# jpe17/TwoTowerMLRetrieval

Hardware: AMD Instinct MI355X
Metric: queries/sec top-k over 10M x 256-d docs (higher is better)
Workload: dtype f32 results (bit-identical to the fp32 FMA chain); f16-MFMA screen + fp32 rescoring; 1 GPU; exact cosine top-10 of B=1024 queries over 10000000 x 256 fp32 unit-norm passages resident in HBM (BASELINE configs[3]; configs[1] batch), row-sharded over 1 GPU(s), screened path (f16-MFMA filter + exact fp32 rescoring, bit-identical to the fp32 kernel); n_docs=10000000, dim=256, batch=1024, k=10, parallelism=rowshard1

## Files before the change

### twotowermlretrieval_amd/csrc/score_topk.hip

```cpp
#include "tt_common.h"

#include <limits.h>
#include <math.h>

namespace {

constexpr int TILE_DOCS = 32;
constexpr int SLAB_BYTES = 32 * 128;
constexpr int NSTAGE = 4;
#ifndef TT_K4_NT_NSTAGE
#define TT_K4_NT_NSTAGE 4
#endif
constexpr int NSTAGE_NT = TT_K4_NT_NSTAGE;
constexpr int WPB = 4;
constexpr int DMA_PER_SLAB = 4;
constexpr int PACE_R = 16;
constexpr int PACE_POLLS = 400;
constexpr int DRAW_POLLS = 1 << 16;
constexpr int DRAW_GAVE_UP = 0x7fffffff;

typedef __attribute__((address_space(3))) void lds_void;
typedef const __attribute__((address_space(1))) void gbl_void;

struct Cand;
// ... 692 lines not shown
            float bv;
            int64_t bi;
            pool_next_best(pool_v, pool_i, n, pv, pi, red_v, red_i, bv, bi);
            if (bi == INT64_MAX)
                break;
            if (tid == 0) {
                top_v[r] = bv;
                top_i[r] = bi;
            }
            pv = bv;
            pi = bi;
            kept = r + 1;
        }
        __syncthreads();
        if (tid < kept) {
            pool_v[tid] = top_v[tid];
            pool_i[tid] = top_i[tid];
        }
        if (tid == 0)
            pool_n = kept;
        __syncthreads();
        return kept;
    };

    for (int base = 0; base < M; base += MERGE_SEG) {
        if (pool_n + MERGE_SEG > MERGE_POOL)
            reduce_pool();
        const int end = min(base + MERGE_SEG, M);
        int64_t ci[MERGE_SEG / MERGE_THREADS];
#pragma unroll
        for (int u = 0; u < MERGE_SEG / MERGE_THREADS; ++u) {
            const int m = base + tid + u * MERGE_THREADS;
            ci[u] = m < end ? ix_at(m) : -1;
        }
#pragma unroll
        for (int u = 0; u < MERGE_SEG / MERGE_THREADS; ++u) {
            if (ci[u] >= 0) {
                const int slot = atomicAdd(&pool_n, 1);
                pool_v[slot] = v_at(base + tid + u * MERGE_THREADS);
                pool_i[slot] = ci[u];
            }
        }
        __syncthreads();
    }
    const int kept = reduce_pool();
    if (tid < k) {
        out_val[(size_t)b * k + tid] = tid < kept ? pool_v[tid] : -INFINITY;
        out_idx[(size_t)b * k + tid] = tid < kept ? pool_i[tid] : -1;
    }
}

__device__ __forceinline__ unsigned order_key(float f)
{
    const unsigned b = __float_as_uint(f);
    return (b & 0x80000000u) ? ~b : (b | 0x80000000u);
}

__device__ __forceinline__ float order_key_to_float(unsigned key)
{
    return __uint_as_float((key & 0x80000000u) ? (key & 0x7fffffffu) : ~key);
}

__global__ __launch_bounds__(256) void kth_largest_kernel(const float *__restrict__ vals, int M, int k,
                                                          float *__restrict__ out, const int *run_if,
                                                          float *__restrict__ top_out)
{
    if (run_if && run_if[blockIdx.x >> 5] == 0)
        return;
    __shared__ int hist[256];
    __shared__ int sel[2];
    __shared__ int wpos;
    const int row = blockIdx.x, tid = threadIdx.x, lane = tid & 63;
    const float *v = vals + (size_t)row * M;
    if (M < k) {
        if (tid == 0 && out)
            out[row] = -INFINITY;
        if (top_out)
            for (int i = tid; i < k; i += 256)
                top_out[(size_t)row * k + i] = i < M ? v[i] : -INFINITY;
        return;
    }
    unsigned prefix = 0u, mask = 0u;
    int k_rem = k;
    constexpr int KTH_REG = 16;
    const bool in_regs = M <= 256 * KTH_REG;
    unsigned keys[KTH_REG];
    if (in_regs) {
#pragma unroll
        for (int i = 0; i < KTH_REG; ++i) {
            const int m = tid + 256 * i;
            keys[i] = m < M ? order_key(v[m]) : 0u;
        }
    }
#pragma unroll 1
    for (int pass = 0; pass < 4; ++pass) {
        const int shift = 24 - 8 * pass;
        hist[tid] = 0;
        __syncthreads();
        if (in_regs) {
#pragma unroll
            for (int i = 0; i < KTH_REG; ++i)
                if (tid + 256 * i < M && (keys[i] & mask) == prefix)
                    atomicAdd(&hist[(keys[i] >> shift) & 255u], 1);
        } else {
            for (int m = tid; m < M; m += 256) {
                const unsigned key = order_key(v[m]);
                if ((key & mask) == prefix)
                    atomicAdd(&hist[(key >> shift) & 255u], 1);
            }
        }
        __syncthreads();
        if (tid < 64) {
            int c[4], s = 0;
#pragma unroll
            for (int i = 0; i < 4; ++i) {
                c[i] = hist[255 - (lane * 4 + i)];
                s += c[i];
            }
            int incl = s;
#pragma unroll
            for (int off = 1; off < 64; off <<= 1) {
                const int y = __shfl_up(incl, off);
                if (lane >= off)
                    incl += y;
            }
            int above = incl - s;
#pragma unroll
            for (int i = 0; i < 4; ++i) {
                if (above < k_rem && above + c[i] >= k_rem) {
                    sel[0] = 255 - (lane * 4 + i);
                    sel[1] = above;
                }
                above += c[i];
            }
        }
        __syncthreads();
        prefix |= (unsigned)sel[0] << shift;
        mask |= 0xffu << shift;
        k_rem -= sel[1];
        __syncthreads();
    }
    const float kth = order_key_to_float(prefix);
    if (tid == 0 && out)
        out[row] = kth;
    if (top_out) {
        if (tid == 0)
            wpos = 0;
        __syncthreads();
        float *dst = top_out + (size_t)row * k;
        if (in_regs) {
#pragma unroll
            for (int i = 0; i < KTH_REG; ++i)
                if (tid + 256 * i < M && keys[i] > prefix)
                    dst[atomicAdd(&wpos, 1)] = order_key_to_float(keys[i]);
        } else {
            for (int m = tid; m < M; m += 256)
                if (order_key(v[m]) > prefix)
                    dst[atomicAdd(&wpos, 1)] = v[m];
        }
        for (int i = k - k_rem + tid; i < k; i += 256)
            dst[i] = kth;
    }
}

__global__ __launch_bounds__(256) void score_rank_kernel(const float *__restrict__ Q,
                                                         const float *__restrict__ D, int N, int d,
                                                         const int64_t *__restrict__ target,
// ... 389 lines not shown
TT_EXPORT size_t tt_score_topk_redo_flags_offset(int B, int64_t N, int d, int k)
{
    if (B <= 0 || N <= 0 || k <= 0)
        return (size_t)-1;
    const Plan pl = make_plan(B, N, k, d);
    return (pl.paced && pl.main.tail_blocks > 0) ? pl.redo_off : (size_t)-1;
}

TT_EXPORT size_t tt_score_topk_workspace_bytes(int B, int64_t N, int d, int k)
{
    if (B <= 0 || N < 0 || k <= 0)
        return 0;
    return make_plan(B, N, k, d).ws_bytes;
}

TT_EXPORT size_t tt_score_topk_bf16_workspace_bytes(int B, int64_t N, int d, int k)
{
    if (B <= 0 || N < 0 || k <= 0)
        return 0;
    return make_plan(B, N, k, d, true).ws_bytes;
}

TT_EXPORT int tt_score_topk_partials_f32(const float *Q, int B, int d, const float *D, int64_t N, int k,
                                         int64_t idx_offset, void *workspace, size_t workspace_bytes,
                                         const float **part_val, const int64_t **part_idx, int *part_m,
                                         void *const *prof_events, tt_stream_t stream)
{
    Plan pl;
    int rc = score_partials(Q, B, d, D, false, N, k, idx_offset, workspace, workspace_bytes, (hipStream_t)stream, &pl,
                            "tt_score_topk_partials_f32", nullptr, prof_events);
    if (rc != TT_OK)
        return rc;
    if (part_val)
        *part_val = (const float *)((const char *)workspace + pl.pval_off);
    if (part_idx)
        *part_idx = (const int64_t *)((const char *)workspace + pl.pidx_off);
    if (part_m)
        *part_m = pl.main.n_chunks * k;
    return TT_OK;
}

namespace {
__global__ __launch_bounds__(64) void redo_flag_kernel(const int64_t *__restrict__ out_idx, int B, int k, int *__restrict__ flags)
{
    const int q = blockIdx.x * 32 + threadIdx.x;
    const bool bad = threadIdx.x < 32 && q < B && out_idx[(size_t)q * k] >= (int64_t)TT_TOPK_INVALID_INDEX;
    const unsigned long long any = __ballot(bad);
    if (threadIdx.x == 0)
        flags[blockIdx.x] = any != 0ull;
}
}

namespace {
int score_topk_pred(const float *Q, int B, int d, const void *D, bool bf16, int64_t N, int k, int64_t idx_offset,
                    float *out_val, int64_t *out_idx, void *workspace, size_t workspace_bytes, const int *run_if,
                    hipStream_t st, const char *who)
{
    if (B < 0 || N < 0 || k <= 0)
        return tt_fail(TT_ERR_BAD_SHAPE, "%s: B=%d N=%lld k=%d", who, B, (long long)N, k);
    if (B == 0)
        return TT_OK;
    if (!score_dim_ok(d, bf16))
        return tt_fail(TT_ERR_UNSUPPORTED, "%s: d=%d (supported: %s)", who, d, score_dims(bf16));
    if (k > 64)
        return tt_fail(TT_ERR_UNSUPPORTED, "%s: k=%d > 64", who, k);
    if (!out_val || !out_idx)
        return tt_fail(TT_ERR_BAD_SHAPE, "%s: null output pointer", who);
    if (N == 0) {
        hipLaunchKernelGGL(topk_merge_kernel, dim3(B), dim3(MERGE_THREADS), 0, st, (const float *)nullptr,
                           (const int64_t *)nullptr, 0, k, out_val, out_idx, (const int *)nullptr, 1, (size_t)0);
        TT_LAUNCH_CHECK();
        return TT_OK;
    }
    Plan pl;
    int rc = score_partials(Q, B, d, D, bf16, N, k, idx_offset, workspace, workspace_bytes, st, &pl, who, run_if);
    if (rc != TT_OK)
        return rc;
    const char *ws = (const char *)workspace;
    hipLaunchKernelGGL(topk_merge_kernel, dim3(B), dim3(MERGE_THREADS), 0, st, (const float *)(ws + pl.pval_off),
                       (const int64_t *)(ws + pl.pidx_off), pl.main.n_chunks * k, k, out_val, out_idx, run_if,
                       pl.main.n_chunks * k, (size_t)0);
    TT_LAUNCH_CHECK();
    if (!run_if && pl.paced && pl.main.tail_blocks > 0 && tt_score_pacing()) {
        int *redo = (int *)((char *)workspace + pl.redo_off);
        hipLaunchKernelGGL(redo_flag_kernel, dim3(pl.main.n_qtiles), dim3(64), 0, st, (const int64_t *)out_idx, B, k, redo);
        TT_LAUNCH_CHECK();
        return score_topk_pred(Q, B, d, D, bf16, N, k, idx_offset, out_val, out_idx, workspace, workspace_bytes, redo, st,
                               who);
    }
    return TT_OK;
}
}

int tt_score_topk_f32_pred(const float *Q, int B, int d, const float *D, int64_t N, int k, int64_t idx_offset,
                           float *out_val, int64_t *out_idx, void *workspace, size_t workspace_bytes,
                           const int *run_if, hipStream_t st)
{
    return score_topk_pred(Q, B, d, D, false, N, k, idx_offset, out_val, out_idx, workspace, workspace_bytes, run_if, st,
                           "tt_score_topk_f32");
}

int tt_score_topk_bf16_pred(const float *Q, int B, int d, const void *D, int64_t N, int k, int64_t idx_offset,
                            float *out_val, int64_t *out_idx, void *workspace, size_t workspace_bytes,
                            const int *run_if, hipStream_t st)
{
    return score_topk_pred(Q, B, d, D, true, N, k, idx_offset, out_val, out_idx, workspace, workspace_bytes, run_if, st,
                           "tt_score_topk_bf16");
}

TT_EXPORT int tt_score_topk_f32(const float *Q, int B, int d, const float *D, int64_t N, int k,
                                int64_t idx_offset, float *out_val, int64_t *out_idx, void *workspace,
                                size_t workspace_bytes, tt_stream_t stream)
{
    return tt_score_topk_f32_pred(Q, B, d, D, N, k, idx_offset, out_val, out_idx, workspace, workspace_bytes, nullptr,
                                  (hipStream_t)stream);
}

TT_EXPORT int tt_score_topk_bf16(const float *Q, int B, int d, const void *D_bf16, int64_t N, int k,
                                 int64_t idx_offset, float *out_val, int64_t *out_idx, void *workspace,
                                 size_t workspace_bytes, tt_stream_t stream)
{
    return tt_score_topk_bf16_pred(Q, B, d, D_bf16, N, k, idx_offset, out_val, out_idx, workspace, workspace_bytes,
                                   nullptr, (hipStream_t)stream);
}

int tt_kth_largest(const float *vals, int B, int M, int k, float *out, hipStream_t st)
{
    hipLaunchKernelGGL(kth_largest_kernel, dim3(B), dim3(256), 0, st, vals, M, k, out, (const int *)nullptr, (float *)nullptr);
    TT_LAUNCH_CHECK();
    return TT_OK;
}

int tt_k_largest_list(const float *vals, int B, int M, int k, float *list, hipStream_t st)
{
    hipLaunchKernelGGL(kth_largest_kernel, dim3(B), dim3(256), 0, st, vals, M, k, (float *)nullptr, (const int *)nullptr, list);
    TT_LAUNCH_CHECK();
    return TT_OK;
}

namespace {
__global__ __launch_bounds__(64) void seed_union_kernel(const float *__restrict__ lists, int world, int B, int ks, int kth,
                                                        float *__restrict__ seed)
{
    const int q = blockIdx.x, lane = threadIdx.x;
    const int M = world * ks;
    __shared__ float v[512];
    for (int i = lane; i < M; i += 64)
        v[i] = lists[((size_t)(i / ks) * B + q) * ks + (i % ks)];
    __syncthreads();
    for (int i = lane; i < M; i += 64) {
        const float x = v[i];
        int before = 0;
        for (int j = 0; j < M; ++j)
            before += (v[j] > x) || (v[j] == x && j < i);
        if (before == kth - 1)
            seed[q] = x;
    }
}
}

TT_EXPORT int tt_seed_union_f32(const float *lists, int world, int B, int list_len, int kth, float *seed, tt_stream_t stream)
{
    if (!lists || !seed || world < 1 || B <= 0 || list_len < 1 || (int64_t)world * list_len > 512 || kth < 1 ||
        kth > world * list_len)
        return tt_fail(TT_ERR_BAD_SHAPE, "tt_seed_union_f32: world=%d B=%d list_len=%d kth=%d (kth <= world * list_len <= 512)",
                       world, B, list_len, kth);
    hipLaunchKernelGGL(seed_union_kernel, dim3(B), dim3(64), 0, (hipStream_t)stream, lists, world, B, list_len, kth, seed);
    TT_LAUNCH_CHECK();
// ... 747 lines not shown
```

### twotowermlretrieval_amd/csrc/screen.hip

```cpp
#include "tt_common.h"
#include <cmath>

#include <hip/hip_fp16.h>
#include <limits.h>
#include <math.h>

int tt_score_topk_f32_pred(const float *Q, int B, int d, const float *D, int64_t N, int k, int64_t idx_offset,
                           float *out_val, int64_t *out_idx, void *workspace, size_t workspace_bytes,
                           const int *run_if, hipStream_t st);
int tt_score_topk_bf16_pred(const float *Q, int B, int d, const void *D, int64_t N, int k, int64_t idx_offset,
                            float *out_val, int64_t *out_idx, void *workspace, size_t workspace_bytes,
                            const int *run_if, hipStream_t st);

int tt_kth_largest(const float *vals, int B, int M, int k, float *out, hipStream_t st);
int tt_k_largest_list(const float *vals, int B, int M, int k, float *list, hipStream_t st);

namespace {

typedef _Float16 h8 __attribute__((ext_vector_type(8)));
typedef _Float16 h4 __attribute__((ext_vector_type(4)));
typedef unsigned u32x4 __attribute__((ext_vector_type(4)));
typedef __attribute__((address_space(3))) void lds_void;
typedef const __attribute__((address_space(1))) void gbl_void;

// ... 69 lines not shown

__device__ __forceinline__ void scand_store_async(const SCand *base, unsigned byte_off, float v, int x)
{
    const unsigned long long bits = ((unsigned long long)(unsigned)x << 32) | (unsigned long long)__float_as_uint(v);
    asm volatile("global_store_dwordx2 %0, %1, %2\n\ts_nop 1" ::"v"(byte_off), "v"(bits), "s"(base) : "memory");
}

__device__ __forceinline__ void f32_store_async(float *dst, float v)
{
    asm volatile("global_store_dword %0, %1, off\n\ts_nop 0" ::"v"(dst), "v"(v) : "memory");
}

constexpr int SQUART = SCAP / 4;
constexpr int SQ_TRIGGER = SQUART - 10;
constexpr int SQ_KEEP_MAX = 4 * SQ_TRIGGER - 4;

__device__ __forceinline__ void screen_compact(SCand *base, const int (&n)[4], int k, float slack, int lane, int &n_new,
                                               float &thr_new, bool &have, bool &overflow)
{
    float v[2];
    int x[2], rank[2];
    bool live[2];
#pragma unroll
    for (int i = 0; i < 2; ++i) {
        v[i] = -INFINITY;
        x[i] = INT_MAX;
        rank[i] = 0;
        live[i] = (lane & 31) < ((lane >> 5) ? n[2 * i + 1] : n[2 * i]);
        if (live[i]) {
            const SCand c = scand_load_l2(base + 64 * i + lane);
            v[i] = c.v;
            x[i] = c.x;
        }
    }
#pragma unroll
    for (int i2 = 0; i2 < 2; ++i2) {
#pragma unroll
        for (int sub = 0; sub < 2; ++sub) {
            const int lim = n[2 * i2 + sub];
            for (int l2 = 0; l2 < lim; ++l2) {
                const float sv = __builtin_bit_cast(float, __builtin_amdgcn_readlane(__builtin_bit_cast(int, v[i2]), 32 * sub + l2));
                const int sx = __builtin_amdgcn_readlane(x[i2], 32 * sub + l2);
#pragma unroll
                for (int i = 0; i < 2; ++i)
                    rank[i] += (sv > v[i] || (sv == v[i] && sx < x[i])) ? 1 : 0;
            }
        }
    }
    const int total = n[0] + n[1] + n[2] + n[3];
    have = total >= k;
    overflow = false;
    n_new = total;
    thr_new = -INFINITY;
    if (have) {
        float kth = -INFINITY;
#pragma unroll
        for (int i = 0; i < 2; ++i) {
            const unsigned long long bk = __ballot(live[i] && rank[i] == k - 1);
            if (bk)
                kth = __builtin_bit_cast(float, __builtin_amdgcn_readlane(__builtin_bit_cast(int, v[i]), __ffsll((long long)bk) - 1));
        }
        thr_new = kth - slack;
        n_new = 0;
#pragma unroll
        for (int i = 0; i < 2; ++i)
            n_new += __popcll(__ballot(live[i] && v[i] >= thr_new));
        if (n_new > SQ_KEEP_MAX) {
            overflow = true;
            n_new = k;
        }
    }
#pragma unroll
    for (int i = 0; i < 2; ++i)
        if (live[i] && rank[i] < n_new) {
            SCand c;
            c.v = v[i];
            c.x = x[i];
            base[SQUART * (rank[i] & 3) + (rank[i] >> 2)] = c;
        }
}

__global__ __launch_bounds__(128) void q_image_kernel(const float *__restrict__ Q, int B, h8 *__restrict__ img,
                                                      float *__restrict__ qnorm, int *__restrict__ flag, int n_flags,
                                                      int *__restrict__ tail_ctr, int n_ctr)
{
    __shared__ int any_bad[2];
    if (blockIdx.x == 0)
        for (int i = threadIdx.x; i < n_ctr; i += 128)
            tail_ctr[i] = 0;
    const int lane = threadIdx.x & 63, wv = threadIdx.x >> 6;
    const int S = blockIdx.x * 2 + wv;
    const int g = lane >> 4, n = lane & 15;
    const int qrow = 16 * S + n;
    const bool live = qrow < B;
    const float *qp = Q + (size_t)min(qrow, B - 1) * 256 + 8 * g;
    float ss = 0.0f;
    bool bad = false;
#pragma unroll
    for (int s = 0; s < 8; ++s) {
        const f32x4 a = *(const f32x4 *)(qp + 32 * s);
        const f32x4 b = *(const f32x4 *)(qp + 32 * s + 4);
        h8 hv;
#pragma unroll
        for (int e = 0; e < 4; ++e) {
            const float x0 = live ? a[e] : 0.0f, x1 = live ? b[e] : 0.0f;
            ss += x0 * x0 + x1 * x1;
            bad |= !(fabsf(x0) <= 60000.0f) || !(fabsf(x1) <= 60000.0f);
            hv[e] = (_Float16)x0;
            hv[4 + e] = (_Float16)x1;
        }
        img[((size_t)S * 8 + s) * 64 + lane] = hv;
    }
    ss += __shfl_xor(ss, 16);
    ss += __shfl_xor(ss, 32);
    if (g == 0)
        qnorm[qrow] = sqrtf(ss);
    const bool wave_bad = __ballot(bad && live) != 0ull;
    if (lane == 0)
        any_bad[wv] = wave_bad ? 1 : 0;
    __syncthreads();
    if (threadIdx.x == 0 && (int)blockIdx.x < n_flags)
        flag[blockIdx.x] = (any_bad[0] | any_bad[1]) ? 2 : 0;
}

template <bool MAXONLY, int NSET, bool BF = false>
__global__ __launch_bounds__(SW * 64, 2) void screen_kernel(ScreenParams p)
{
    extern __shared__ __attribute__((aligned(16))) char ring[];
    constexpr int DMA_AUX = NSET < 3 ? 2 : 0;
    const int lane = threadIdx.x & 63;
    const int w = __builtin_amdgcn_readfirstlane(threadIdx.x >> 6);
    const int chunk = blockIdx.x % p.n_chunks;
    const int qgroup = blockIdx.x / p.n_chunks;
    int t0 = chunk * p.tiles_per_chunk;
    int t1 = min(t0 + p.tiles_per_chunk, p.static_tiles);
    __shared__ int next_block;
    const int k = p.k;
    const int g = lane >> 4, n = lane & 15;
    constexpr int QW = 16 * NSET, QB = SW * QW;
    const int qbase = qgroup * QB + w * QW;
    const bool wave_live = qbase < p.B;

    h8 qreg[NSET][8];
    float eps2[NSET];
    f32x4 negthr[NSET];
    int cnt[NSET];
#pragma unroll
    for (int c = 0; c < NSET; ++c)
        cnt[c] = 0;
#pragma unroll
    for (int c = 0; c < NSET; ++c) {
        const int qrow = qbase + 16 * c + n;
        const bool live = qrow < p.B;
        float qn = 0.0f;
        if (wave_live) {
            const h8 *src = p.qimg + ((size_t)(qbase / 16 + c) * 8) * 64 + lane;
#pragma unroll
            for (int s = 0; s < 8; ++s)
                qreg[c][s] = src[s * 64];
            qn = p.qnorm[qrow];
        }
        eps2[c] = 2.0f * screen_eps(qn, p.dmax);
        const float floor_thr = -(1.01f * qn * p.dmax + 1e-30f);
        const float t_init = live ? ((!MAXONLY && p.thr0) ? fmaxf(p.thr0[(size_t)qrow * p.thr0_stride + p.thr0_stride - 1] - eps2[c], floor_thr)
                                                    : floor_thr)
                            : INFINITY;
        float c_init = -t_init;
        if (MAXONLY)
            c_init = (p.dbg_thr && live) ? -p.dbg_thr[qrow] : 0.0f;
        negthr[c] = f32x4{c_init, c_init, c_init, c_init};
    }

// ... 378 lines not shown
#pragma unroll
                        for (int r = 0; r < 4; ++r)
                            if (tile_base + 16 * u + 4 * g + r >= p.N) {
#pragma unroll
                                for (int c = 0; c < NQS; ++c)
                                    acc[u][c][r] = -INFINITY;
                            }
                }
                int mall = INT_MIN;
#pragma unroll
                for (int u = 0; u < 2; ++u)
#pragma unroll
                    for (int c = 0; c < NQS; ++c)
#pragma unroll
                        for (int r = 0; r < 4; ++r)
                            mall = max(mall, __float_as_int(acc[u][c][r]));
                if (__ballot(mall >= 0) != 0ull) {
#pragma unroll
                    for (int c = 0; c < NQS; ++c) {
                        const unsigned mine = (unsigned)(((16 * c + n) * SCAP + SQUART * g) * sizeof(SCand));
                        const float thr_c = -negthr[c][0];
#pragma unroll
                        for (int u = 0; u < 2; ++u)
#pragma unroll
                            for (int r = 0; r < 4; ++r) {
                                if (__float_as_int(acc[u][c][r]) >= 0) {
                                    scand_store_async(cwave, mine + (unsigned)cnt[c] * (unsigned)sizeof(SCand),
                                                      acc[u][c][r] + thr_c, tile_base + 16 * u + 4 * g + r);
                                    ++cnt[c];
                                }
                            }
                        unsigned long long full = __ballot(cnt[c] > SQ_TRIGGER);
                        full = (full | (full >> 32));
                        full = (full | (full >> 16)) & 0xffffull;
                        if (full)
                            compact_where(c, (unsigned)full);
                    }
                }
            } else {
#pragma unroll
                for (int c = 0; c < NQS; ++c) {
                    float m = -INFINITY;
#pragma unroll
                    for (int u = 0; u < 2; ++u)
#pragma unroll
                        for (int r = 0; r < 4; ++r)
                            m = fmaxf(m, (!partial || tile_base + 16 * u + 4 * g + r < p.N) ? acc[u][c][r] : -INFINITY);
                    m = fmaxf(m, __shfl_xor(m, 16));
                    m = fmaxf(m, __shfl_xor(m, 32));
                    const int qrow = qbase + 16 * c + n;
                    if (g == 0 && qrow < p.B)
                        f32_store_async(p.max_val + (size_t)qrow * p.n_tiles + tile, m);
                }
            }
        }
    }
    asm volatile("s_waitcnt vmcnt(0)" ::: "memory");
    if (MAXONLY)
        return;
#pragma unroll
    for (int c = 0; c < NQS; ++c) {
        int tot = cnt[c] + __shfl_xor(cnt[c], 16);
        tot += __shfl_xor(tot, 32);
        const unsigned long long over = __ballot(tot > k) & 0xffffull;
        if (over)
            compact_where(c, (unsigned)over);
        int packed = cnt[c] << (8 * g);
        packed |= __shfl_xor(packed, 16);
        packed |= __shfl_xor(packed, 32);
        const int qrow = qbase + 16 * c + n;
        if (g == 0 && qrow < p.B)
            p.pcnt[(size_t)qrow * p.n_chunks + chunk] = packed;
    }
}

struct FinishParams {
    const float *Q;
    const float *D32;
    const unsigned *Dbf;
    int B, N, k, n_chunks;
    float dmax;
    const SCand *cand;
    const int *pcnt;
    int *flag;
    int64_t idx_offset;
    float *out_val;
    int64_t *out_idx;
    int q_per_block;
    int *stats;
};

__device__ __forceinline__ bool before_f(float sa, int ia, float sb, int ib) { return sa > sb || (sa == sb && ia < ib); }

__device__ __forceinline__ unsigned f32_order_key(float f)
{
    const unsigned b = __float_as_uint(f);
    return (b & 0x80000000u) ? ~b : (b | 0x80000000u);
}
__device__ __forceinline__ float f32_from_order_key(unsigned k)
{
    return __uint_as_float((k & 0x80000000u) ? (k & 0x7fffffffu) : ~k);
}

__global__ __launch_bounds__(256) void screen_finish_kernel(FinishParams p)
{
    __shared__ float pool_v[POOL_MAX];
    __shared__ float qs[256];
    __shared__ float sv_v[SURV_MAX];
    __shared__ int sv_x[SURV_MAX];
    __shared__ float red_v[4];
    __shared__ int hist[256];
    extern __shared__ int fin_dyn[];
    int *const ccnt = fin_dyn;
    int *const pre = fin_dyn + p.n_chunks;
    __shared__ int sel[2];
    __shared__ int n_pool, n_surv;
    const int row = blockIdx.x, tid = threadIdx.x;
    if (tid == 0)
        n_pool = n_surv = 0;
    qs[tid] = p.Q[(size_t)row * 256 + tid];
    __syncthreads();
    float ss = qs[tid] * qs[tid];
#pragma unroll
    for (int off = 32; off >= 1; off >>= 1)
        ss += __shfl_xor(ss, off);
    if ((tid & 63) == 0)
        red_v[tid >> 6] = ss;
    __syncthreads();
    const float eps2 = 2.0f * screen_eps(sqrtf(red_v[0] + red_v[1] + red_v[2] + red_v[3]), p.dmax);
    __syncthreads();

    const int qgroup = row / p.q_per_block, qin = row % p.q_per_block;
    bool too_many = false;
    const int per = (p.n_chunks + 255) / 256;
    {
        int sum = 0;
        for (int c = tid * per; c < min(tid * per + per, p.n_chunks); ++c) {
            const int v = p.pcnt[(size_t)row * p.n_chunks + c];
            ccnt[c] = v;
            sum += (v & 0xff) + ((v >> 8) & 0xff) + ((v >> 16) & 0xff) + ((v >> 24) & 0xff);
        }
        int inc = sum;
#pragma unroll
        for (int off = 1; off < 64; off <<= 1) {
            const int v = __shfl_up(inc, off);
            if ((tid & 63) >= off)
                inc += v;
        }
        if ((tid & 63) == 63)
            hist[tid >> 6] = inc;
        __syncthreads();
        int base = 0;
        for (int wv = 0; wv < (tid >> 6); ++wv)
            base += hist[wv];
        if (tid == 255)
            n_pool = base + inc;
        __syncthreads();
        hist[tid] = base + inc - sum;
    }
    __syncthreads();
    {
        int run = hist[tid];
        for (int c = tid * per; c < min(tid * per + per, p.n_chunks); ++c) {
            pre[c] = run;
            const int v = ccnt[c];
            run += (v & 0xff) + ((v >> 8) & 0xff) + ((v >> 16) & 0xff) + ((v >> 24) & 0xff);
        }
        if (tid == 255)
            pre[p.n_chunks] = n_pool;
    }
    __syncthreads();
    const int total = n_pool;
    if (total > POOL_MAX)
        too_many = true;
    auto locate = [&](int m) -> const SCand * {
        int lo = 0, hi = p.n_chunks;
        while (hi - lo > 1) {
            const int mid = (lo + hi) >> 1;
            if (pre[mid] <= m)
                lo = mid;
            else
                hi = mid;
        }
        int o = m - pre[lo], slot = 0;
#pragma unroll
        for (int gq = 0; gq < 4; ++gq) {
            const int ng = (ccnt[lo] >> (8 * gq)) & 0xff;
            if (o >= 0 && o < ng)
                slot = SQUART * gq + o;
            o -= ng;
            if (o < 0)
                o = INT_MIN / 2;
        }
        return p.cand + ((size_t)(qgroup * p.n_chunks + lo) * p.q_per_block + qin) * SCAP + slot;
    };
    for (int m = tid; m < total && m < POOL_MAX; m += 256)
        pool_v[m] = locate(m)->v;
    __syncthreads();
    const int np = min(n_pool, POOL_MAX);
    float kth = -INFINITY;
    const int found = np >= p.k ? p.k : np;
    if (np >= p.k) {
        unsigned prefix = 0u, mask = 0u;
        int k_rem = p.k;
#pragma unroll 1
        for (int pass = 0; pass < 4; ++pass) {
            const int shift = 24 - 8 * pass;
            hist[tid] = 0;
            __syncthreads();
            for (int m = tid; m < np; m += 256) {
                const unsigned key = f32_order_key(pool_v[m]);
                if ((key & mask) == prefix)
// ... 273 lines not shown
}

template <bool MAXONLY, bool BF>
const void *screen_fn(bool stream, int q_per_block, int nset)
{
    if (stream)
        return q_per_block == 64 ? (const void *)screen_stream_kernel<MAXONLY, 4, BF>
                                 : (const void *)screen_stream_kernel<MAXONLY, 2, BF>;
    switch (nset) {
    case 4: return (const void *)screen_kernel<MAXONLY, 4, BF>;
    case 3: return (const void *)screen_kernel<MAXONLY, 3, BF>;
    case 2: return (const void *)screen_kernel<MAXONLY, 2, BF>;
    default: return (const void *)screen_kernel<MAXONLY, 1, BF>;
    }
}

int launch_screen(bool stream, int q_per_block, int nset, bool maxonly, ScreenParams p, int n_tasks, hipStream_t st,
                  bool bf16 = false)
{
    const void *fn = maxonly ? (bf16 ? screen_fn<true, true>(stream, q_per_block, nset) : screen_fn<true, false>(stream, q_per_block, nset))
                             : (bf16 ? screen_fn<false, true>(stream, q_per_block, nset) : screen_fn<false, false>(stream, q_per_block, nset));
    const size_t lds = stream ? (size_t)TW * TSTAGE * TSLAB_BYTES : (size_t)SRING * STILE_BYTES;
    const int blocks = stream ? (n_tasks + TW - 1) / TW : n_tasks;
    TT_HIP_CHECK(hipFuncSetAttribute(fn, hipFuncAttributeMaxDynamicSharedMemorySize, (int)lds));
    void *args[] = {&p};
    TT_HIP_CHECK(hipLaunchKernel(fn, dim3(blocks), dim3((stream ? TW : SW) * 64), args, lds, st));
    return TT_OK;
}

}

TT_EXPORT int tt_index_build_f16(const float *D, int64_t N, int d, void *D16, float *stats, tt_stream_t stream)
{
    if (N < 0 || d <= 0 || (d & 3))
        return tt_fail(TT_ERR_BAD_SHAPE, "tt_index_build_f16: N=%lld d=%d", (long long)N, d);
    if (!stats || (N > 0 && (!D || !D16)))
        return tt_fail(TT_ERR_BAD_SHAPE, "tt_index_build_f16: null pointer");
    hipStream_t st = (hipStream_t)stream;
    TT_RC_CHECK(tt_zero_async(stats, 2 * sizeof(float), st));
    if (N == 0)
        return TT_OK;
    const int64_t want_blocks = (N + 3) / 4;
    hipLaunchKernelGGL(build_f16_kernel, dim3((unsigned)(want_blocks > 8192 ? 8192 : want_blocks)), dim3(256), 0, st, D,
                       N, d, (_Float16 *)D16, (unsigned *)stats);
    TT_LAUNCH_CHECK();
    return TT_OK;
}

TT_EXPORT int tt_index_build_from_bf16(const void *D_bf16, int64_t N, int d, float *D32, void *D16, float *stats,
                                       int reset_stats, tt_stream_t stream)
{
    if (N < 0 || d <= 0 || (d & 3))
        return tt_fail(TT_ERR_BAD_SHAPE, "tt_index_build_from_bf16: N=%lld d=%d", (long long)N, d);
    if (N > 0 && (!D_bf16 || !D32))
        return tt_fail(TT_ERR_BAD_SHAPE, "tt_index_build_from_bf16: null pointer");
    hipStream_t st = (hipStream_t)stream;
    if (stats && reset_stats)
        TT_RC_CHECK(tt_zero_async(stats, 2 * sizeof(float), st));
    if (N == 0)
        return TT_OK;
    const int64_t want_blocks = (N + 3) / 4;
    hipLaunchKernelGGL(build_from_bf16_kernel, dim3((unsigned)(want_blocks > 8192 ? 8192 : want_blocks)), dim3(256), 0,
                       st, (const unsigned short *)D_bf16, N, d, D32, (_Float16 *)D16, (unsigned *)stats);
    TT_LAUNCH_CHECK();
    return TT_OK;
}

TT_EXPORT size_t tt_score_topk_screened_workspace_bytes(int B, int64_t N, int d, int k)
{
    if (B <= 0 || N <= 0)
        return 0;
    return make_splan(B, N, k).ws_bytes + tt_score_topk_workspace_bytes(B, N, d, k);
}

TT_EXPORT size_t tt_score_topk_screened_stats_offset(int B, int64_t N, int d, int k)
{
    (void)d;
    if (B <= 0 || N <= 0)
        return 0;
    return make_splan(B, N, k).stats_off;
}

namespace {
__global__ void seed_fill_kernel(float *seed, int n)
{
    const int i = blockIdx.x * 256 + threadIdx.x;
    if (i < n)
        seed[i] = -3.0e38f;
}

enum class Phase {
    Whole,
    SeedThreshold,
    SeedList,
    Seeded,
};

int screened_impl(const char *who, Phase phase, const float *Q, int B, int d, const void *D32, const void *D16, int64_t N, int k,
                  int k_seed, float dmax_norm, int64_t idx_offset, float *out_val, int64_t *out_idx, int32_t *fallback_flag,
                  float *seed, void *workspace, size_t workspace_bytes, void *const *prof_events, hipStream_t st,
                  bool bf16 = false)
{
    if (B <= 0 || N <= 0 || k <= 0)
        return tt_fail(TT_ERR_BAD_SHAPE, "%s: B=%d N=%lld k=%d", who, B, (long long)N, k);
    if (d != 256)
        return tt_fail(TT_ERR_UNSUPPORTED, "%s: d=%d (supported: 256)", who, d);
    if (k > 64)
        return tt_fail(TT_ERR_UNSUPPORTED, "%s: k=%d > 64", who, k);
    if (N >= (int64_t)INT_MAX - 64)
        return tt_fail(TT_ERR_UNSUPPORTED, "%s: N too large; shard the corpus", who);
    if (!(dmax_norm >= 0.0f) || !(dmax_norm < 60000.0f))
        return tt_fail(TT_ERR_UNSUPPORTED, "%s: corpus norm %g outside the fp16 range", who, dmax_norm);
    const bool seed_only = phase == Phase::SeedThreshold || phase == Phase::SeedList;
    const bool caller_seed = phase == Phase::Seeded;
    if (!Q || !D16 || !fallback_flag || (!seed_only && (!D32 || !out_val || !out_idx)) || (phase != Phase::Whole && !seed))
        return tt_fail(TT_ERR_BAD_SHAPE, "%s: null pointer", who);
    if (seed_only && (k_seed < 1 || k_seed > k))
        return tt_fail(TT_ERR_BAD_SHAPE, "%s: k_seed=%d outside [1, k=%d]", who, k_seed, k);
    const SPlan pl = make_splan(B, N, k);
    const size_t need = pl.ws_bytes + (bf16 ? tt_score_topk_bf16_workspace_bytes(B, N, d, k) : tt_score_topk_workspace_bytes(B, N, d, k));
    if (!workspace || workspace_bytes < need || ((uintptr_t)workspace & 255) || (bf16 && ((uintptr_t)D16 & 15)))
        return tt_fail(TT_ERR_WORKSPACE, "%s: workspace %zu < %zu bytes", who, workspace_bytes, need);
    char *ws = (char *)workspace;
    const int k_thr = phase == Phase::SeedThreshold ? k_seed : k;
    float *thr_out = phase == Phase::SeedThreshold ? seed : (float *)(ws + pl.sthr_val_off);

    ScreenParams sp;
    sp.Q = Q;
    sp.D16 = (const _Float16 *)D16;
    sp.B = B;
    sp.N = (int)N;
    sp.k = k;
    sp.n_chunks = pl.n_chunks;
    sp.tiles_per_chunk = pl.tiles_per_chunk;
    sp.n_tiles = pl.n_tiles;
    sp.static_tiles = pl.static_tiles;
    sp.tail_g = pl.tail_g;
    sp.tail_blocks = pl.tail_blocks;
    sp.tail_ctr = (int *)(ws + pl.tailctr_off);
    sp.dmax = dmax_norm;
    sp.cand = (SCand *)(ws + pl.cand_off);
    sp.pcnt = (int *)(ws + pl.pcnt_off);
    sp.flag = fallback_flag;
    sp.max_val = nullptr;
    sp.thr0 = nullptr;
    sp.thr0_stride = k;
    sp.qimg = (const h8 *)(ws + pl.qimg_off);
    sp.qnorm = (const float *)(ws + pl.qnorm_off);
    sp.dbg_thr = nullptr;
    if (caller_seed) {
        sp.thr0 = seed;
        sp.thr0_stride = 1;
    } else {
        hipLaunchKernelGGL(q_image_kernel, dim3(pl.rows_pad / 32), dim3(128), 0, st, Q, B, (h8 *)(ws + pl.qimg_off),
                           (float *)(ws + pl.qnorm_off), fallback_flag, (B + 31) / 32, (int *)(ws + pl.tailctr_off),
                           pl.n_qgroups);
        TT_LAUNCH_CHECK();
        if (pl.sample) {
            ScreenParams ss = sp;
            ss.N = (int)pl.s_docs;
            ss.n_tiles = pl.s_tiles;
            ss.n_chunks = pl.s_chunks;
            ss.tiles_per_chunk = pl.s_tiles_per_chunk;
            ss.static_tiles = pl.s_tiles;
            ss.tail_blocks = 0;
            ss.max_val = (float *)(ws + pl.smax_val_off);
            TT_RC_CHECK(launch_screen(pl.stream, pl.q_per_block, pl.nset, true, ss, pl.n_qgroups * pl.s_chunks, st, bf16));
            if (phase == Phase::SeedList)
                TT_RC_CHECK(tt_k_largest_list(ss.max_val, B, pl.s_tiles, k_seed, seed, st));
            else
                TT_RC_CHECK(tt_kth_largest(ss.max_val, B, pl.s_tiles, k_thr, thr_out, st));
            sp.thr0 = (const float *)(ws + pl.sthr_val_off);
            sp.thr0_stride = 1;
        } else if (seed_only) {
            const int n = phase == Phase::SeedList ? B * k_seed : B;
            hipLaunchKernelGGL(seed_fill_kernel, dim3((n + 255) / 256), dim3(256), 0, st, seed, n);
            TT_LAUNCH_CHECK();
        }
    }
    if (seed_only)
        return TT_OK;
    if (prof_events)
        TT_HIP_CHECK(hipEventRecord((hipEvent_t)prof_events[0], st));
    TT_RC_CHECK(launch_screen(pl.stream, pl.q_per_block, pl.nset, false, sp, pl.n_qgroups * pl.n_chunks, st, bf16));
    if (prof_events)
        TT_HIP_CHECK(hipEventRecord((hipEvent_t)prof_events[1], st));

    FinishParams fp;
    fp.Q = Q;
    fp.D32 = bf16 ? nullptr : (const float *)D32;
    fp.Dbf = bf16 ? (const unsigned *)D32 : nullptr;
    fp.B = B;
    fp.N = (int)N;
    fp.k = k;
    fp.n_chunks = pl.n_chunks;
    fp.q_per_block = pl.q_per_block;
    fp.dmax = dmax_norm;
    fp.cand = sp.cand;
    fp.pcnt = sp.pcnt;
    fp.flag = fallback_flag;
    fp.idx_offset = idx_offset;
    fp.out_val = out_val;
    fp.out_idx = out_idx;
    fp.stats = (int *)(ws + pl.stats_off);
    hipLaunchKernelGGL(screen_finish_kernel, dim3(B), dim3(256), (size_t)(2 * pl.n_chunks + 1) * sizeof(int), st, fp);
    TT_LAUNCH_CHECK();
    if (bf16)
        return tt_score_topk_bf16_pred(Q, B, d, D32, N, k, idx_offset, out_val, out_idx, ws + pl.ws_bytes,
                                       workspace_bytes - pl.ws_bytes, fallback_flag, st);
    return tt_score_topk_f32_pred(Q, B, d, (const float *)D32, N, k, idx_offset, out_val, out_idx, ws + pl.ws_bytes,
                                  workspace_bytes - pl.ws_bytes, fallback_flag, st);
}
}

TT_EXPORT size_t tt_score_topk_screened_bf16_workspace_bytes(int B, int64_t N, int d, int k)
{
    if (B <= 0 || N <= 0)
        return 0;
    return make_splan(B, N, k).ws_bytes + tt_score_topk_bf16_workspace_bytes(B, N, d, k);
}

TT_EXPORT int tt_index_stats_bf16(const void *D_bf16, int64_t N, int d, float *stats, int reset_stats, tt_stream_t stream)
{
    hipStream_t st = (hipStream_t)stream;
    if (N < 0 || d <= 0 || d % 4 != 0 || d > 4096)
        return tt_fail(TT_ERR_BAD_SHAPE, "tt_index_stats_bf16: N=%lld d=%d", (long long)N, d);
    if (!stats || (N > 0 && !D_bf16))
        return tt_fail(TT_ERR_BAD_SHAPE, "tt_index_stats_bf16: null pointer");
    if (reset_stats)
        TT_RC_CHECK(tt_zero_async(stats, 2 * sizeof(float), st));
    if (N == 0)
        return TT_OK;
    const int64_t want_blocks = (N + 3) / 4;
    hipLaunchKernelGGL(build_from_bf16_kernel, dim3((unsigned)(want_blocks > 8192 ? 8192 : want_blocks)), dim3(256), 0,
                       st, (const unsigned short *)D_bf16, N, d, (float *)nullptr, (_Float16 *)nullptr, (unsigned *)stats);
    TT_LAUNCH_CHECK();
    return TT_OK;
}

TT_EXPORT int tt_score_topk_screened_bf16(const float *Q, int B, int d, const void *D_bf16, int64_t N, int k, float dmax_norm,
                                          int64_t idx_offset, float *out_val, int64_t *out_idx, int32_t *fallback_flag,
                                          void *workspace, size_t workspace_bytes, void *const *prof_events, tt_stream_t stream)
{
    return screened_impl("tt_score_topk_screened_bf16", Phase::Whole, Q, B, d, D_bf16, D_bf16, N, k, k, dmax_norm, idx_offset,
                         out_val, out_idx, fallback_flag, nullptr, workspace, workspace_bytes, prof_events, (hipStream_t)stream,
                         true);
}

TT_EXPORT int tt_score_topk_screened_seed_list_bf16(const float *Q, int B, int d, const void *D_bf16, int64_t N, int k,
                                                    int k_seed, float dmax_norm, int32_t *fallback_flag, float *seed_list,
                                                    void *workspace, size_t workspace_bytes, tt_stream_t stream)
{
    return screened_impl("tt_score_topk_screened_seed_list_bf16", Phase::SeedList, Q, B, d, nullptr, D_bf16, N, k, k_seed,
                         dmax_norm, 0, nullptr, nullptr, fallback_flag, seed_list, workspace, workspace_bytes, nullptr,
                         (hipStream_t)stream, true);
}

TT_EXPORT int tt_score_topk_screened_seeded_bf16(const float *Q, int B, int d, const void *D_bf16, int64_t N, int k,
                                                 float dmax_norm, int64_t idx_offset, float *out_val, int64_t *out_idx,
                                                 int32_t *fallback_flag, const float *seed, void *workspace,
                                                 size_t workspace_bytes, void *const *prof_events, tt_stream_t stream)
{
    return screened_impl("tt_score_topk_screened_seeded_bf16", Phase::Seeded, Q, B, d, D_bf16, D_bf16, N, k, k, dmax_norm,
                         idx_offset, out_val, out_idx, fallback_flag, (float *)seed, workspace, workspace_bytes, prof_events,
                         (hipStream_t)stream, true);
}

TT_EXPORT int tt_score_topk_screened_f32(const float *Q, int B, int d, const float *D32, const void *D16, int64_t N,
                                         int k, float dmax_norm, int64_t idx_offset, float *out_val, int64_t *out_idx,
                                         int32_t *fallback_flag, void *workspace, size_t workspace_bytes,
                                         void *const *prof_events, tt_stream_t stream)
{
    return screened_impl("tt_score_topk_screened_f32", Phase::Whole, Q, B, d, D32, D16, N, k, k, dmax_norm, idx_offset, out_val, out_idx,
                         fallback_flag, nullptr, workspace, workspace_bytes, prof_events, (hipStream_t)stream);
}

TT_EXPORT int tt_score_topk_screened_seed_f32(const float *Q, int B, int d, const void *D16, int64_t N, int k, int k_seed,
                                              float dmax_norm, int32_t *fallback_flag, float *seed, void *workspace,
                                              size_t workspace_bytes, tt_stream_t stream)
{
    return screened_impl("tt_score_topk_screened_seed_f32", Phase::SeedThreshold, Q, B, d, nullptr, D16, N, k, k_seed, dmax_norm, 0, nullptr, nullptr,
                         fallback_flag, seed, workspace, workspace_bytes, nullptr, (hipStream_t)stream);
// ... 7 lines not shown
                         nullptr, fallback_flag, seed_list, workspace, workspace_bytes, nullptr, (hipStream_t)stream);
}

TT_EXPORT int tt_score_topk_screened_seeded_f32(const float *Q, int B, int d, const float *D32, const void *D16, int64_t N,
                                                int k, float dmax_norm, int64_t idx_offset, float *out_val, int64_t *out_idx,
                                                int32_t *fallback_flag, const float *seed, void *workspace,
                                                size_t workspace_bytes, void *const *prof_events, tt_stream_t stream)
{
    return screened_impl("tt_score_topk_screened_seeded_f32", Phase::Seeded, Q, B, d, D32, D16, N, k, k, dmax_norm, idx_offset, out_val,
                         out_idx, fallback_flag, (float *)seed, workspace, workspace_bytes, prof_events, (hipStream_t)stream);
}


namespace {
struct DbgPlan {
    int q_per_block, n_qgroups, rows_pad, n_tiles, n_chunks, tiles_per_chunk;
    size_t qimg_off, qnorm_off, flag_off, total;
};
bool make_dbg_plan(int B, int64_t N, int form, DbgPlan &pl)
{
    if (form != 0 && form != 1 && form != 2 && form != 4)
        return false;
    pl.q_per_block = form == 0 ? 32 : SW * 16 * form;
    pl.n_qgroups = (B + pl.q_per_block - 1) / pl.q_per_block;
    pl.rows_pad = pl.n_qgroups * pl.q_per_block;
    pl.n_tiles = (int)((N + 31) / 32);
    const TTChunks c = tt_chunks(pl.n_tiles, one_round(form == 0, pl.n_qgroups), INT_MAX);
    pl.tiles_per_chunk = c.tiles_per_chunk;
    pl.n_chunks = c.n_chunks;
    TTWorkspace ws;
    pl.qimg_off = ws.take((size_t)pl.rows_pad * 256 * sizeof(_Float16));
    pl.qnorm_off = ws.take((size_t)pl.rows_pad * sizeof(float));
    pl.flag_off = ws.take((size_t)(pl.rows_pad / 32 + 1) * sizeof(int));
    pl.total = ws.off;
    return true;
}
}

TT_EXPORT size_t tt_debug_screen_s16_workspace_bytes(int B, int64_t N, int form)
{
    DbgPlan pl;
    if (B <= 0 || N <= 0 || !make_dbg_plan(B, N, form, pl))
        return 0;
    return pl.total;
}

namespace {
int debug_screen(const float *Q, int B, const void *D16, int64_t N, float dmax_norm, const float *thr, int form, float *out_t,
                 void *workspace, size_t workspace_bytes, tt_stream_t stream, bool bf16)
{
    hipStream_t st = (hipStream_t)stream;
    DbgPlan pl;
    if (B <= 0 || N <= 0 || N >= (int64_t)INT_MAX - 64 || !make_dbg_plan(B, N, form, pl))
        return tt_fail(TT_ERR_BAD_SHAPE, "tt_debug_screen_s16: B=%d N=%lld form=%d", B, (long long)N, form);
    if (!Q || !D16 || !out_t)
        return tt_fail(TT_ERR_BAD_SHAPE, "tt_debug_screen_s16: null pointer");
    if (!workspace || workspace_bytes < pl.total || ((uintptr_t)workspace & 255))
        return tt_fail(TT_ERR_WORKSPACE, "tt_debug_screen_s16: workspace %zu < %zu bytes", workspace_bytes, pl.total);
    char *ws = (char *)workspace;
    ScreenParams sp;
    sp.Q = Q;
    sp.D16 = (const _Float16 *)D16;
    sp.B = B;
    sp.N = (int)N;
    sp.k = 1;
    sp.n_chunks = pl.n_chunks;
    sp.tiles_per_chunk = pl.tiles_per_chunk;
    sp.n_tiles = pl.n_tiles;
    sp.static_tiles = pl.n_tiles;
    sp.tail_g = 1;
    sp.tail_blocks = 0;
    sp.tail_ctr = nullptr;
    sp.dmax = dmax_norm;
    sp.cand = nullptr;
    sp.pcnt = nullptr;
    sp.flag = (int *)(ws + pl.flag_off);
    sp.max_val = out_t;
    sp.thr0 = nullptr;
    sp.thr0_stride = 1;
    sp.qimg = (const h8 *)(ws + pl.qimg_off);
    sp.qnorm = (const float *)(ws + pl.qnorm_off);
    sp.dbg_thr = thr;
    hipLaunchKernelGGL(q_image_kernel, dim3(pl.rows_pad / 32), dim3(128), 0, st, Q, B, (h8 *)(ws + pl.qimg_off),
                       (float *)(ws + pl.qnorm_off), sp.flag, pl.rows_pad / 32, (int *)nullptr, 0);
    TT_LAUNCH_CHECK();
    return launch_screen(form == 0, pl.q_per_block, form, true, sp, pl.n_qgroups * pl.n_chunks, st, bf16);
}
}

TT_EXPORT int tt_debug_screen_s16(const float *Q, int B, const void *D16, int64_t N, float dmax_norm, const float *thr,
                                  int form, float *out_t, void *workspace, size_t workspace_bytes, tt_stream_t stream)
{
    return debug_screen(Q, B, D16, N, dmax_norm, thr, form, out_t, workspace, workspace_bytes, stream, false);
}

TT_EXPORT int tt_debug_screen_s16_bf16(const float *Q, int B, const void *D_bf16, int64_t N, float dmax_norm, const float *thr,
                                       int form, float *out_t, void *workspace, size_t workspace_bytes, tt_stream_t stream)
{
    return debug_screen(Q, B, D_bf16, N, dmax_norm, thr, form, out_t, workspace, workspace_bytes, stream, true);
}
```

Before: 254,700 queries/s.

## Fold seed fill into q_image, reuse qnorm in finish, trim finish LDS

Folds the separate seed-fill kernel into q_image_kernel so one launch does both. The finish kernel now reads the query norm q_image already computed instead of doing its own block reduction and two syncs. It also aliases the survivor-value buffer onto the pool buffer so the kernel fits four blocks per CU. It raises the kth-largest register capacity from 16 to 20 keys per thread and adds a guard for the redo-flag grid size. Together these cut launch and sync overhead and raise occupancy, at the cost of more registers in the kth kernel and a norm that may not exactly match the old in-kernel reduction.

```diff
diff --git a/twotowermlretrieval_amd/csrc/score_topk.hip b/twotowermlretrieval_amd/csrc/score_topk.hip
--- a/twotowermlretrieval_amd/csrc/score_topk.hip
+++ b/twotowermlretrieval_amd/csrc/score_topk.hip
@@ -798,7 +798,7 @@
     }
     unsigned prefix = 0u, mask = 0u;
     int k_rem = k;
-    constexpr int KTH_REG = 16;
+    constexpr int KTH_REG = 20;
     const bool in_regs = M <= 256 * KTH_REG;
     unsigned keys[KTH_REG];
     if (in_regs) {
@@ -1354,8 +1354,11 @@
                        pl.main.n_chunks * k, (size_t)0);
     TT_LAUNCH_CHECK();
     if (!run_if && pl.paced && pl.main.tail_blocks > 0 && tt_score_pacing()) {
+        const int n_flags = (B + 31) / 32;
+        if (pl.main.n_qtiles != n_flags)
+            return tt_fail(TT_ERR_UNSUPPORTED, "%s: paced plan with %d query tiles for %d redo flags", who, pl.main.n_qtiles, n_flags);
         int *redo = (int *)((char *)workspace + pl.redo_off);
-        hipLaunchKernelGGL(redo_flag_kernel, dim3(pl.main.n_qtiles), dim3(64), 0, st, (const int64_t *)out_idx, B, k, redo);
+        hipLaunchKernelGGL(redo_flag_kernel, dim3(n_flags), dim3(64), 0, st, (const int64_t *)out_idx, B, k, redo);
         TT_LAUNCH_CHECK();
         return score_topk_pred(Q, B, d, D, bf16, N, k, idx_offset, out_val, out_idx, workspace, workspace_bytes, redo, st,
                                who);
diff --git a/twotowermlretrieval_amd/csrc/screen.hip b/twotowermlretrieval_amd/csrc/screen.hip
--- a/twotowermlretrieval_amd/csrc/screen.hip
+++ b/twotowermlretrieval_amd/csrc/screen.hip
@@ -175,12 +175,15 @@
 
 __global__ __launch_bounds__(128) void q_image_kernel(const float *__restrict__ Q, int B, h8 *__restrict__ img,
                                                       float *__restrict__ qnorm, int *__restrict__ flag, int n_flags,
-                                                      int *__restrict__ tail_ctr, int n_ctr)
+                                                      int *__restrict__ tail_ctr, int n_ctr, float *__restrict__ seed,
+                                                      int n_seed)
 {
     __shared__ int any_bad[2];
     if (blockIdx.x == 0)
         for (int i = threadIdx.x; i < n_ctr; i += 128)
             tail_ctr[i] = 0;
+    for (int i = blockIdx.x * 128 + threadIdx.x; i < n_seed; i += gridDim.x * 128)
+        seed[i] = -3.0e38f;
     const int lane = threadIdx.x & 63, wv = threadIdx.x >> 6;
     const int S = blockIdx.x * 2 + wv;
     const int g = lane >> 4, n = lane & 15;
@@ -725,6 +728,7 @@
     float dmax;
     const SCand *cand;
     const int *pcnt;
+    const float *qnorm;
     int *flag;
     int64_t idx_offset;
     float *out_val;
@@ -749,10 +753,11 @@
 {
     __shared__ float pool_v[POOL_MAX];
     __shared__ float qs[256];
-    __shared__ float sv_v[SURV_MAX];
     __shared__ int sv_x[SURV_MAX];
-    __shared__ float red_v[4];
     __shared__ int hist[256];
+    static_assert(SURV_MAX <= POOL_MAX, "sv_v aliases pool_v");
+    float *const sv_v = pool_v;
+    static_assert(sizeof(float) * (POOL_MAX + 256) + sizeof(int) * (SURV_MAX + 256 + 4 + 2 * 252 + 1) <= 40 * 1024, "four per CU");
     extern __shared__ int fin_dyn[];
     int *const ccnt = fin_dyn;
     int *const pre = fin_dyn + p.n_chunks;
@@ -762,15 +767,7 @@
     if (tid == 0)
         n_pool = n_surv = 0;
     qs[tid] = p.Q[(size_t)row * 256 + tid];
-    __syncthreads();
-    float ss = qs[tid] * qs[tid];
-#pragma unroll
-    for (int off = 32; off >= 1; off >>= 1)
-        ss += __shfl_xor(ss, off);
-    if ((tid & 63) == 0)
-        red_v[tid >> 6] = ss;
-    __syncthreads();
-    const float eps2 = 2.0f * screen_eps(sqrtf(red_v[0] + red_v[1] + red_v[2] + red_v[3]), p.dmax);
+    const float eps2 = 2.0f * screen_eps(p.qnorm[row], p.dmax);
     __syncthreads();
 
     const int qgroup = row / p.q_per_block, qin = row % p.q_per_block;
@@ -1210,13 +1207,6 @@
 }
 
 namespace {
-__global__ void seed_fill_kernel(float *seed, int n)
-{
-    const int i = blockIdx.x * 256 + threadIdx.x;
-    if (i < n)
-        seed[i] = -3.0e38f;
-}
-
 enum class Phase {
     Whole,
     SeedThreshold,
@@ -1280,9 +1270,10 @@
         sp.thr0 = seed;
         sp.thr0_stride = 1;
     } else {
+        const int n_fill = pl.sample || !seed_only ? 0 : (phase == Phase::SeedList ? B * k_seed : B);
         hipLaunchKernelGGL(q_image_kernel, dim3(pl.rows_pad / 32), dim3(128), 0, st, Q, B, (h8 *)(ws + pl.qimg_off),
                            (float *)(ws + pl.qnorm_off), fallback_flag, (B + 31) / 32, (int *)(ws + pl.tailctr_off),
-                           pl.n_qgroups);
+                           pl.n_qgroups, seed, n_fill);
         TT_LAUNCH_CHECK();
         if (pl.sample) {
             ScreenParams ss = sp;
@@ -1300,10 +1291,6 @@
                 TT_RC_CHECK(tt_kth_largest(ss.max_val, B, pl.s_tiles, k_thr, thr_out, st));
             sp.thr0 = (const float *)(ws + pl.sthr_val_off);
             sp.thr0_stride = 1;
-        } else if (seed_only) {
-            const int n = phase == Phase::SeedList ? B * k_seed : B;
-            hipLaunchKernelGGL(seed_fill_kernel, dim3((n + 255) / 256), dim3(256), 0, st, seed, n);
-            TT_LAUNCH_CHECK();
         }
     }
     if (seed_only)
@@ -1326,6 +1313,7 @@
     fp.dmax = dmax_norm;
     fp.cand = sp.cand;
     fp.pcnt = sp.pcnt;
+    fp.qnorm = sp.qnorm;
     fp.flag = fallback_flag;
     fp.idx_offset = idx_offset;
     fp.out_val = out_val;
@@ -1499,7 +1487,7 @@
     sp.qnorm = (const float *)(ws + pl.qnorm_off);
     sp.dbg_thr = thr;
     hipLaunchKernelGGL(q_image_kernel, dim3(pl.rows_pad / 32), dim3(128), 0, st, Q, B, (h8 *)(ws + pl.qimg_off),
-                       (float *)(ws + pl.qnorm_off), sp.flag, pl.rows_pad / 32, (int *)nullptr, 0);
+                       (float *)(ws + pl.qnorm_off), sp.flag, pl.rows_pad / 32, (int *)nullptr, 0, (float *)nullptr, 0);
     TT_LAUNCH_CHECK();
     return launch_screen(form == 0, pl.q_per_block, form, true, sp, pl.n_qgroups * pl.n_chunks, st, bf16);
 }
```

Result: no change. 255,600 queries/s, median of 6 (+0.4%).
